# CLIAI/speaker-diarization-toolkit

Hardware: AMD Instinct MI355X
Metric: segment-embeddings/sec (higher is better)
Workload: dtype bf16; 1 GPU; config #2: 1k synthetic 2-s segments/GPU -> fbank -> ECAPA-TDNN C=1024 -> L2 -> cosine argmax vs 100 profiles; segments_per_gpu=1000, embed_dim=192, weights=random-init seed 0 (20.77 M params), parallelism=segments sharded x1, profiles replicated

## Files before the change

### speaker-diarization-toolkit_amd/csrc/common.hpp

```cpp
#pragma once
#include <hip/hip_runtime.h>
#include <stdint.h>
#include <stdio.h>
#include <vector>

#include "../../include/sdk_hip.h"

typedef __bf16 bf16_t;
typedef __bf16 bf16x8 __attribute__((ext_vector_type(8)));
typedef __bf16 bf16x4 __attribute__((ext_vector_type(4)));
typedef __bf16 bf16x2 __attribute__((ext_vector_type(2)));
typedef float f32x4 __attribute__((ext_vector_type(4)));
typedef float f32x16 __attribute__((ext_vector_type(16)));
typedef uint32_t u32x4 __attribute__((ext_vector_type(4)));
typedef uint32_t u32x2 __attribute__((ext_vector_type(2)));

struct sdk_prof_rec {
  int family;
  hipEvent_t a, b;
  double flops, bytes;
};
struct sdk_ctx {
  int device;
  int num_cu;
  hipDeviceProp_t prop;
  bool prof_on = false;
  bool no_chain_fusion = false;
  bool no_chain_two_per_cu = false;
  bool no_chain_packed = false;
  bool no_asp_packed = false;
  bool no_asp_seg = false;
  bool no_h_kblocked = false;
  int precision = 0;
  int aff_fast = 1;
  void* dbg_ptr = nullptr;
  void* gemm_clk_ptr = nullptr;
  void* gemm_stamps_ptr = nullptr;
  int hp_gemm_variant = 0;
  int matvec_variant = 0;
  int aff_boundary_pen = 0;
  int chol_pivot_rtol_ppb = 1000;
  int chol_shift_ppb = 0;
  bool ahc_distances_only = false;
  bool snorm_scores_only = false;
  int aff_variant = 0;
  std::vector<const void*> lds_optin;
  std::vector<sdk_prof_rec> prof;
};

int sdk_lds_optin(sdk_ctx* ctx, const void* func, int bytes);

int asp_fused_launch(sdk_ctx* ctx, const uint16_t* ah, int64_t ldah, const uint16_t* w2, const uint16_t* w2p, const float* b2,
                     const uint16_t* h, int64_t ldh, int B, int T, int C, int A, float* pooled, void* stream, bool kblocked = false, bool f16 = false);

int se_gate_residual_impl(sdk_ctx* ctx, const uint16_t* z, int64_t ldz, const uint16_t* x, int64_t ldx, const float* w1t, const float* b1, const float* w2t,
                          const float* b2, uint16_t* out, int64_t ldo, int B, int T, int C, int Cse, const float* mean_in, void* ws, size_t ws_bytes,
                          void* stream, bool f16);
int asp_stats_impl(sdk_ctx* ctx, const uint16_t* h, int64_t ldh, int B, int T, int C, float* out_ctx, void* stream, bool f16);
int asp_pool_impl(sdk_ctx* ctx, const float* logits, int64_t ldl, const uint16_t* h, int64_t ldh, int B, int T, int C, float* pooled, void* stream, bool f16);

int res2net_chain_launch(sdk_ctx* ctx, const uint16_t* U, int64_t ldu, uint16_t* R, int64_t ldr, const uint16_t* const* W,
                         const uint16_t* const* Wpk, const float* const* bias, const float* const* scale, const float* const* shift,
                         int nconv, int B, int T, int dil, void* stream, bool f16 = false);

int resnet_tstp_impl(sdk_ctx* ctx, const uint16_t* x, int B, int F, int T, int C, float* out, void* stream, bool f16);
int resnet_masked_tstp_impl(sdk_ctx* ctx, const uint16_t* x, int B, int F, int T, int C, int S, const float* w, const int32_t* valid, float* out,
                            void* stream, bool f16);
int resnet_zero_invalid_impl(sdk_ctx* ctx, float* emb, int n, int dim, const int32_t* valid, void* stream);

size_t ahc_workspace_bytes(const int32_t* offsets, int G);
int ahc_launch(sdk_ctx* ctx, const float* E, int ldE, int dim, const int32_t* offsets, int G, double* Z, int32_t* status, void* ws, void* stream);

struct ProfScope {
  sdk_ctx* c; hipStream_t s; size_t slot; bool on;
  ProfScope(sdk_ctx* ctx, void* stream, int family, double flops, double bytes) : c(ctx), s((hipStream_t)stream), slot(0), on(ctx && ctx->prof_on) {
    if (!on) return;
    sdk_prof_rec r{family, nullptr, nullptr, flops, bytes};
    (void)hipEventCreate(&r.a); (void)hipEventCreate(&r.b);
    (void)hipEventRecord(r.a, s);
    slot = c->prof.size();
    c->prof.push_back(r);
  }
  ~ProfScope() { if (on) (void)hipEventRecord(c->prof[slot].b, s); }
};

void sdk_set_error(const char* fmt, ...) __attribute__((format(printf, 1, 2)));

#define SDK_HIP_OK(expr)                                                              \
  do {                                                                                \
    hipError_t _e = (expr);                                                           \
    if (_e != hipSuccess) {                                                           \
      sdk_set_error("%s failed: %s (%s:%d)", #expr, hipGetErrorString(_e), __FILE__, __LINE__); \
      return 1;                                                                       \
    }                                                                                 \
  } while (0)

#define SDK_REQUIRE(cond, ...)            \
  do {                                    \
    if (!(cond)) {                        \
      sdk_set_error(__VA_ARGS__);         \
      return 2;                           \
    }                                     \
  } while (0)

#define SDK_LAUNCH_CHECK()                                                         \
  do {                                                                             \
    hipError_t _e = hipGetLastError();                                             \
    if (_e != hipSuccess) {                                                        \
      sdk_set_error("kernel launch failed: %s (%s:%d)", hipGetErrorString(_e), __FILE__, __LINE__); \
      return 1;                                                                    \
    }                                                                              \
  } while (0)

static inline int ceil_div(int a, int b) { return (a + b - 1) / b; }

__device__ __forceinline__ float bf16_to_f32(bf16_t v) { return (float)v; }
__device__ __forceinline__ bf16_t f32_to_bf16(float v) { return (bf16_t)v; }

__device__ __forceinline__ float bf16_bits_to_f32(uint32_t lo16) { return __uint_as_float(lo16 << 16); }

__device__ __forceinline__ void unpack8(const u32x4& v, float* f) {
#pragma unroll
  for (int i = 0; i < 4; ++i) {
    f[2 * i] = __uint_as_float(v[i] << 16);
    f[2 * i + 1] = __uint_as_float(v[i] & 0xffff0000u);
  }
}
__device__ __forceinline__ uint32_t pack2(float a, float b) {
  bf16x2 t;
  t[0] = (bf16_t)a;
  t[1] = (bf16_t)b;
  return __builtin_bit_cast(uint32_t, t);
}
typedef _Float16 f16x8_t __attribute__((ext_vector_type(8)));
typedef _Float16 f16x2_t __attribute__((ext_vector_type(2)));
__device__ __forceinline__ float sat_f16(float a) {
  const float c = fminf(fmaxf(a, -65504.f), 65504.f);
  return a != a ? a : c;
}
template <bool F16>
__device__ __forceinline__ uint32_t pack2t(float a, float b) {
  if constexpr (F16) {
    f16x2_t t;
    t[0] = (_Float16)sat_f16(a);
    t[1] = (_Float16)sat_f16(b);
    return __builtin_bit_cast(uint32_t, t);
  } else {
    return pack2(a, b);
  }
}
template <bool F16>
__device__ __forceinline__ void unpack8t(const u32x4& v, float* f) {
  if constexpr (F16) {
#pragma unroll
    for (int i = 0; i < 4; ++i) {
      const uint32_t w = v[i];
      const f16x2_t t = __builtin_bit_cast(f16x2_t, w);
      f[2 * i] = (float)t[0];
      f[2 * i + 1] = (float)t[1];
    }
  } else {
    unpack8(v, f);
  }
}

__device__ __forceinline__ u32x4 pack8(const float* f) {
  u32x4 v;
#pragma unroll
  for (int i = 0; i < 4; ++i) v[i] = pack2(f[2 * i], f[2 * i + 1]);
  return v;
}
template <bool F16>
__device__ __forceinline__ u32x4 pack8t(const float* f) {
  u32x4 v;
#pragma unroll
  for (int i = 0; i < 4; ++i) v[i] = pack2t<F16>(f[2 * i], f[2 * i + 1]);
  return v;
}
template <bool F16>
__device__ __forceinline__ float load1t(const bf16_t* q) {
  if constexpr (F16) return (float)*reinterpret_cast<const _Float16*>(q);
  else return bf16_to_f32(*q);
}
template <bool F16>
__device__ __forceinline__ f32x4 mfma_16x16x32(bf16x8 a, bf16x8 b, f32x4 c) {
  if constexpr (F16) return __builtin_amdgcn_mfma_f32_16x16x32_f16(__builtin_bit_cast(f16x8_t, a), __builtin_bit_cast(f16x8_t, b), c, 0, 0, 0);
  else return __builtin_amdgcn_mfma_f32_16x16x32_bf16(a, b, c, 0, 0, 0);
}
template <bool F16>
__device__ __forceinline__ f32x16 mfma_32x32x16(bf16x8 a, bf16x8 b, f32x16 c) {
  if constexpr (F16) return __builtin_amdgcn_mfma_f32_32x32x16_f16(__builtin_bit_cast(f16x8_t, a), __builtin_bit_cast(f16x8_t, b), c, 0, 0, 0);
  else return __builtin_amdgcn_mfma_f32_32x32x16_bf16(a, b, c, 0, 0, 0);
}

__device__ __forceinline__ float wave_sum(float v) {
#pragma unroll
  for (int o = 32; o > 0; o >>= 1) v += __shfl_xor(v, o, 64);
  return v;
// ... 25 lines not shown
```

### speaker-diarization-toolkit_amd/csrc/fbank.hip

```cpp
#include <math.h>
#include <string.h>

#include <type_traits>

#include "common.hpp"
#include "hp.hpp"

namespace {

constexpr int NFFT = 400, HOP = 160, NMEL = 80, NBIN = 201;
constexpr int FT = 32;
constexpr int NW = 7;
constexpr int NSYM = 208;
constexpr int KSTEPS = NSYM / 16;
constexpr int TILE_SAMPLES = (FT - 1) * HOP + NFFT;
constexpr int AROW = NSYM + 8;
constexpr int PW_STRIDE = NW * 32 + 1;
constexpr int MELW_MAX = 512;

struct FbankTables {
  uint16_t dft[NW][2][KSTEPS][2][64][8];
  int32_t mstart[NMEL];
  int32_t mlen[NMEL];
  int32_t moff[NMEL];
  float melw[MELW_MAX];
  uint16_t dft16[NW][2][KSTEPS][2][64][8];
};

template <bool F16>
__global__ __launch_bounds__(NW * 64) __attribute__((amdgpu_waves_per_eu(4, 4))) void fbank_tile_kernel(const int16_t* __restrict__ pcm, int S, int T,
                                                            int tiles_per_seg, const FbankTables* __restrict__ tab,
                                                            float* __restrict__ L, unsigned long long* __restrict__ dbg,
                                                            const int32_t* __restrict__ starts, int64_t n_total) {
  __shared__ __attribute__((aligned(16))) char lds[4 * FT * AROW * 2 + TILE_SAMPLES * 4];
  int nstamp = 0;
  auto stamp = [&]() { if (dbg && threadIdx.x == 0 && blockIdx.x < 256) dbg[blockIdx.x * 16 + nstamp++] = __builtin_amdgcn_s_memrealtime(); };
  stamp();
  typedef typename std::conditional<F16, _Float16, bf16_t>::type el_t;
  typedef el_t elx8 __attribute__((ext_vector_type(8)));
  typedef el_t elx2 __attribute__((ext_vector_type(2)));
  el_t* img = reinterpret_cast<el_t*>(lds);
  float* xs = reinterpret_cast<float*>(lds + 4 * FT * AROW * 2);
  float* pw = reinterpret_cast<float*>(lds);
  static_assert(FT * PW_STRIDE * 4 <= 4 * FT * AROW * 2, "power tile must fit over the folded images");
  static_assert((MELW_MAX + 3 * NMEL) * 4 <= TILE_SAMPLES * 4, "mel tables must fit over the raw samples");
  const int tid = threadIdx.x, lane = tid & 63, w = tid >> 6;
  const int b = blockIdx.x / tiles_per_seg;
  const int t0 = (blockIdx.x - b * tiles_per_seg) * FT;
  const int64_t s0 = (int64_t)t0 * HOP - NFFT / 2;
  const int64_t w0 = starts ? (int64_t)starts[b] : (int64_t)b * S;
  const int16_t* seg = pcm + w0;
  const int Sv = starts ? (int)(n_total - w0 < S ? (n_total - w0 < 0 ? 0 : n_total - w0) : S) : S;

  {
    constexpr int NLD = (TILE_SAMPLES + NW * 64 - 1) / (NW * 64);
    int16_t raw[NLD];
#pragma unroll
    for (int i = 0; i < NLD; ++i) {
      const int64_t g = s0 + tid + i * (NW * 64);
      raw[i] = seg[g < 0 ? 0 : (g < Sv ? g : (Sv > 0 ? Sv - 1 : 0))];
    }
#pragma unroll
    for (int i = 0; i < NLD; ++i) {
      const int q = tid + i * (NW * 64);
      const int64_t g = s0 + q;
      if (q < TILE_SAMPLES) xs[q] = (g >= 0 && g < Sv) ? (float)raw[i] * (1.0f / 32768.0f) : 0.f;
    }
  }
  __syncthreads();
  stamp();
  for (int e = tid; e < FT * (NSYM / 2); e += NW * 64) {
    const int i = e / (NSYM / 2), n = (e - i * (NSYM / 2)) * 2;
    float ec[2] = {0.f, 0.f}, es[2] = {0.f, 0.f};
#pragma unroll
    for (int q = 0; q < 2; ++q) {
      const int nn = n + q;
      if (nn <= NFFT / 2) {
        const float xa = xs[i * HOP + nn], xb = xs[i * HOP + (nn == 0 ? 0 : NFFT - nn)];
        ec[q] = xa + xb;
        es[q] = xa - xb;
      }
    }
    const el_t ch0 = (el_t)ec[0], ch1 = (el_t)ec[1], sh0 = (el_t)es[0], sh1 = (el_t)es[1];
    auto pk = [](float a, float b) { elx2 t; t[0] = (el_t)a; t[1] = (el_t)b; return __builtin_bit_cast(uint32_t, t); };
    uint32_t* dst = reinterpret_cast<uint32_t*>(img + i * AROW + n);
    dst[(0 * FT * AROW) / 2] = pk((float)ch0, (float)ch1);
    dst[(1 * FT * AROW) / 2] = pk(ec[0] - (float)ch0, ec[1] - (float)ch1);
    dst[(2 * FT * AROW) / 2] = pk((float)sh0, (float)sh1);
    dst[(3 * FT * AROW) / 2] = pk(es[0] - (float)sh0, es[1] - (float)sh1);
  }
  __syncthreads();
  stamp();

  f32x16 are, aim;
#pragma unroll
  for (int r = 0; r < 16; ++r) { are[r] = 0.f; aim[r] = 0.f; }
  const int fi = lane & 31, kk = lane >> 5;
  const el_t* arow = img + fi * AROW + kk * 8;
  const __amdgpu_buffer_rsrc_t trs = __builtin_amdgcn_make_buffer_rsrc(const_cast<uint16_t*>(F16 ? &tab->dft16[0][0][0][0][0][0] : &tab->dft[0][0][0][0][0][0]), 0, (int)sizeof(tab->dft), 0x00020000);
  const int wu = __builtin_amdgcn_readfirstlane(w);
  elx8 bt[3][4];
  elx8 ac[2][4];
  auto load_b = [&](int ks, elx8* dst) {
#pragma unroll
    for (int v = 0; v < 2; ++v) {
      dst[v] = __builtin_bit_cast(elx8, __builtin_amdgcn_raw_buffer_load_b128(trs, lane * 16, ((((wu * 2 + 0) * KSTEPS + ks) * 2 + v) * 64) * 16, 0));
      dst[2 + v] = __builtin_bit_cast(elx8, __builtin_amdgcn_raw_buffer_load_b128(trs, lane * 16, ((((wu * 2 + 1) * KSTEPS + ks) * 2 + v) * 64) * 16, 0));
    }
  };
  auto load_a = [&](int ks, elx8* dst) {
#pragma unroll
    for (int q = 0; q < 4; ++q) dst[q] = *reinterpret_cast<const elx8*>(arow + (q * FT) * AROW + ks * 16);
  };
  auto mma = [](const elx8& a, const elx8& b, const f32x16& c) {
    if constexpr (F16) return __builtin_amdgcn_mfma_f32_32x32x16_f16(a, b, c, 0, 0, 0);
    else return __builtin_amdgcn_mfma_f32_32x32x16_bf16(a, b, c, 0, 0, 0);
  };
  load_b(0, bt[0]);
  load_b(1, bt[1]);
  load_a(0, ac[0]);
#pragma unroll
  for (int ks = 0; ks < KSTEPS; ++ks) {
    __builtin_amdgcn_sched_barrier(0);
    if (ks + 2 < KSTEPS) load_b(ks + 2, bt[(ks + 2) % 3]);
    if (ks + 1 < KSTEPS) load_a(ks + 1, ac[(ks + 1) & 1]);
    __builtin_amdgcn_sched_barrier(0);
    const elx8* bc = bt[ks % 3];
    const elx8* aa = ac[ks & 1];
    are = mma(aa[1], bc[0], are);
    aim = mma(aa[3], bc[2], aim);
    are = mma(aa[0], bc[1], are);
    aim = mma(aa[2], bc[3], aim);
    are = mma(aa[0], bc[0], are);
    aim = mma(aa[2], bc[2], aim);
  }
  __syncthreads();
#pragma unroll
  for (int r = 0; r < 16; ++r) {
    const int frame = (r & 3) + 8 * (r >> 2) + 4 * kk;
    pw[frame * PW_STRIDE + w * 32 + fi] = are[r] * are[r] + aim[r] * aim[r];
  }
  float* melw = xs;
  int* mtab = reinterpret_cast<int*>(xs + MELW_MAX);
  {
    constexpr int NLD = (MELW_MAX + NW * 64 - 1) / (NW * 64);
    float wv[NLD];
    int tv[3] = {0, 0, 0};
#pragma unroll
    for (int i = 0; i < NLD; ++i) wv[i] = tab->melw[min(tid + i * (NW * 64), MELW_MAX - 1)];
    if (tid < NMEL) { tv[0] = tab->mstart[tid]; tv[1] = tab->mlen[tid]; tv[2] = tab->moff[tid]; }
#pragma unroll
    for (int i = 0; i < NLD; ++i)
      if (tid + i * (NW * 64) < MELW_MAX) melw[tid + i * (NW * 64)] = wv[i];
    if (tid < NMEL) { mtab[tid] = tv[0]; mtab[NMEL + tid] = tv[1]; mtab[2 * NMEL + tid] = tv[2]; }
  }
  __syncthreads();
  stamp();
  for (int o = tid; o < FT * NMEL; o += NW * 64) {
    const int frame = o / NMEL, m = o - frame * NMEL;
    const int t = t0 + frame;
    if (t < T) {
      const int st = mtab[m], ln = mtab[NMEL + m], of = mtab[2 * NMEL + m];
      float acc = 0.f;
      for (int i = 0; i < ln; ++i) acc += pw[frame * PW_STRIDE + st + i] * melw[of + i];
      if constexpr (F16) L[((int64_t)b * T + t) * NMEL + m] = 10.0f * log10f(fmaxf(acc, 1e-10f));
      else L[((int64_t)b * T + t) * NMEL + m] = 3.0102999566398120f * __log2f(fmaxf(acc, 1e-10f));
    }
  }
  stamp();
}

template <bool HP, bool F16 = false>
__global__ __launch_bounds__(256) void fbank_norm_kernel(const float* __restrict__ L, int T, bf16_t* __restrict__ feats,
                                                        int ldf) {
  __shared__ float red[256];
  __shared__ float mean[NMEL];
  const int tid = threadIdx.x;
  const float* Ls = L + (int64_t)blockIdx.x * T * NMEL;
  float mx = -INFINITY;
  for (int i = tid; i < T * NMEL; i += 256) mx = fmaxf(mx, Ls[i]);
  red[tid] = mx;
  __syncthreads();
  for (int o = 128; o > 0; o >>= 1) {
    if (tid < o) red[tid] = fmaxf(red[tid], red[tid + o]);
    __syncthreads();
  }
  const float flo = red[0] - 80.0f;
  __syncthreads();
  const int m = tid % NMEL, g = tid / NMEL;
  const float pv = fmaxf(Ls[m], flo);
  float s = 0.f;
  if (g < 3)
    for (int t = g; t < T; t += 3) s += fmaxf(Ls[t * NMEL + m], flo) - pv;
  red[tid] = s;
  __syncthreads();
  if (tid < NMEL) mean[tid] = pv + (red[tid] + red[tid + NMEL] + red[tid + 2 * NMEL]) / (float)T;
  __syncthreads();
  const int c8n = (HP ? ldf >> 1 : ldf) >> 3;
  bf16_t* out = feats + (int64_t)blockIdx.x * T * ldf;
  for (int i = tid; i < T * c8n; i += 256) {
    const int t = i / c8n, c8 = i - t * c8n;
    float f[8];
#pragma unroll
    for (int e = 0; e < 8; ++e) {
      const int c = c8 * 8 + e;
      f[e] = c < NMEL ? fmaxf(Ls[t * NMEL + c], flo) - mean[c] : 0.f;
    }
    if constexpr (HP) sdk_hp::store8(reinterpret_cast<uint16_t*>(out) + (int64_t)t * ldf + c8 * 8, ldf >> 1, f);
    else *reinterpret_cast<u32x4*>(out + (int64_t)t * ldf + c8 * 8) = pack8t<F16>(f);
  }
}

constexpr int NORM_LDS_MAX_T = 480;
template <bool HP, bool F16 = false>
__global__ __launch_bounds__(256) void fbank_norm_lds_kernel(const float* __restrict__ L, int T, bf16_t* __restrict__ feats,
                                                            int ldf) {
  extern __shared__ __attribute__((aligned(16))) float tile[];
  __shared__ float red[256];
  __shared__ float mean[NMEL];
  const int tid = threadIdx.x;
  const int n4 = T * (NMEL / 4);
  const f32x4* Ls = reinterpret_cast<const f32x4*>(L + (int64_t)blockIdx.x * T * NMEL);
  float mx = -INFINITY;
  constexpr int UN = 8;
  for (int i0 = tid; i0 < n4; i0 += 256 * UN) {
    f32x4 v[UN];
#pragma unroll
    for (int u = 0; u < UN; ++u) v[u] = Ls[min(i0 + 256 * u, n4 - 1)];
#pragma unroll
    for (int u = 0; u < UN; ++u) {
      const int i = i0 + 256 * u;
      if (i < n4) {
        reinterpret_cast<f32x4*>(tile)[i] = v[u];
        mx = fmaxf(fmaxf(mx, fmaxf(v[u][0], v[u][1])), fmaxf(v[u][2], v[u][3]));
      }
    }
  }
  red[tid] = mx;
  __syncthreads();
  for (int o = 128; o > 0; o >>= 1) {
    if (tid < o) red[tid] = fmaxf(red[tid], red[tid + o]);
    __syncthreads();
  }
  const float flo = red[0] - 80.0f;
  __syncthreads();
  const int m = tid % NMEL, g = tid / NMEL;
  const float pv = fmaxf(tile[m], flo);
  float s = 0.f;
  if (g < 3)
    for (int t = g; t < T; t += 3) s += fmaxf(tile[t * NMEL + m], flo) - pv;
  red[tid] = s;
  __syncthreads();
  if (tid < NMEL) mean[tid] = pv + (red[tid] + red[tid + NMEL] + red[tid + 2 * NMEL]) / (float)T;
  __syncthreads();
  const int c8n = (HP ? ldf >> 1 : ldf) >> 3;
  bf16_t* out = feats + (int64_t)blockIdx.x * T * ldf;
  for (int i = tid; i < T * c8n; i += 256) {
    const int t = i / c8n, c8 = i - t * c8n;
    float f[8];
#pragma unroll
    for (int e = 0; e < 8; ++e) {
      const int c = c8 * 8 + e;
      f[e] = c < NMEL ? fmaxf(tile[t * NMEL + c], flo) - mean[c] : 0.f;
    }
    if constexpr (HP) sdk_hp::store8(reinterpret_cast<uint16_t*>(out) + (int64_t)t * ldf + c8 * 8, ldf >> 1, f);
    else *reinterpret_cast<u32x4*>(out + (int64_t)t * ldf + c8 * 8) = pack8t<F16>(f);
  }
}

}

extern "C" size_t sdk_fbank_tables_bytes(void) { return sizeof(FbankTables); }

extern "C" int sdk_fbank_tables_fill(void* host_dst, size_t bytes) {
  SDK_REQUIRE(host_dst && bytes >= sizeof(FbankTables), "sdk_fbank_tables_fill: buffer too small (%zu < %zu)", bytes,
              sizeof(FbankTables));
  FbankTables* t = (FbankTables*)host_dst;
  memset(t, 0, sizeof(FbankTables));
  const double PI = 3.14159265358979323846;
  auto bf16_bits = [](float v) -> uint16_t {
    uint32_t u;
    memcpy(&u, &v, 4);
    return (uint16_t)((u + 0x7FFFu + ((u >> 16) & 1u)) >> 16);
  };
  auto f16_bits = [](double v) -> uint16_t {
    const double a = fabs(v);
    uint16_t out;
    if (a == 0.0) out = 0;
    else {
      int e;
      (void)frexp(a, &e);
      int ex = e - 1;
      if (ex < -14) ex = -14;
      const double q = ldexp(1.0, ex - 10);
      double n = nearbyint(a / q);
      if (n >= 2048.0) { n /= 2.0; ex += 1; }
      const int mant = (int)n;
      out = mant < 1024 ? (uint16_t)mant : (uint16_t)(((ex + 15) << 10) | (mant - 1024));
    }
    return (uint16_t)(out | (v < 0 ? 0x8000u : 0u));
  };
  auto f16_val = [](uint16_t h) -> double {
    const int e = (h >> 10) & 31, m = h & 1023;
    const double a = e ? ldexp(1.0 + m / 1024.0, e - 15) : ldexp((double)m, -24);
    return (h & 0x8000u) ? -a : a;
  };
  auto bf16_val = [](uint16_t b) -> float {
    const uint32_t u = (uint32_t)b << 16;
    float v;
    memcpy(&v, &u, 4);
    return v;
  };
  for (int w = 0; w < NW; ++w)
    for (int ks = 0; ks < KSTEPS; ++ks)
      for (int l = 0; l < 64; ++l)
        for (int j = 0; j < 8; ++j) {
          const int n = ks * 16 + 8 * (l >> 5) + j;
          const int f = w * 32 + (l & 31);
          double vc = 0.0, vs = 0.0;
          if (f < NBIN && n <= NFFT / 2) {
            const double win = 0.54 - 0.46 * cos(2.0 * PI * n / NFFT);
            const double ang = 2.0 * PI * (double)((n * f) % NFFT) / NFFT;
            const double half = (n == 0 || n == NFFT / 2) ? 0.5 : 1.0;
            vc = half * win * cos(ang);
            vs = -win * sin(ang);
          }
          const uint16_t ch = bf16_bits((float)vc), sh = bf16_bits((float)vs);
          t->dft[w][0][ks][0][l][j] = ch;
          t->dft[w][0][ks][1][l][j] = bf16_bits((float)(vc - (double)bf16_val(ch)));
          t->dft[w][1][ks][0][l][j] = sh;
          t->dft[w][1][ks][1][l][j] = bf16_bits((float)(vs - (double)bf16_val(sh)));
          const uint16_t ch16 = f16_bits(vc), sh16 = f16_bits(vs);
          t->dft16[w][0][ks][0][l][j] = ch16;
          t->dft16[w][0][ks][1][l][j] = f16_bits(vc - f16_val(ch16));
          t->dft16[w][1][ks][0][l][j] = sh16;
          t->dft16[w][1][ks][1][l][j] = f16_bits(vs - f16_val(sh16));
        }
  auto hz2mel = [](double f) { return 2595.0 * log10(1.0 + f / 700.0); };
  auto mel2hz = [](double m) { return 700.0 * (pow(10.0, m / 2595.0) - 1.0); };
  double pts[NMEL + 2];
  const double mlo = hz2mel(0.0), mhi = hz2mel(8000.0);
  for (int i = 0; i < NMEL + 2; ++i) pts[i] = mel2hz(mlo + (mhi - mlo) * i / (NMEL + 1));
  int off = 0;
  for (int m = 0; m < NMEL; ++m) {
    const double lo = pts[m], ce = pts[m + 1], hi = pts[m + 2];
    int first = -1, last = -1;
    float wv[NBIN];
    for (int f = 0; f < NBIN; ++f) {
      const double fr = 8000.0 * f / (NBIN - 1);
      const double up = (fr - lo) / (ce - lo), dn = (hi - fr) / (hi - ce);
      const double v = fmax(0.0, fmin(up, dn));
      wv[f] = (float)v;
      if (v > 0.0) {
        if (first < 0) first = f;
        last = f;
      }
    }
    t->mstart[m] = first < 0 ? 0 : first;
    t->mlen[m] = first < 0 ? 0 : last - first + 1;
    t->moff[m] = off;
    SDK_REQUIRE(off + t->mlen[m] <= MELW_MAX, "sdk_fbank_tables_fill: mel table overflow");
    for (int i = 0; i < t->mlen[m]; ++i) t->melw[off + i] = wv[first + i];
    off += t->mlen[m];
  }
  return 0;
}

extern "C" size_t sdk_fbank_workspace_bytes(int B, int S) {
  if (B <= 0 || S <= 0) return 0;
  return (size_t)B * (size_t)(1 + S / HOP) * NMEL * sizeof(float);
}

static int fbank_launch(sdk_ctx* ctx, const int16_t* pcm, const int32_t* starts, int64_t n_total, int B, int S, const void* tabs, uint16_t* feats,
                        int ldf, void* ws, size_t ws_bytes, int precision, void* stream, const char* who) {
  SDK_REQUIRE(ctx && pcm && tabs && feats && ws, "%s: null argument", who);
  SDK_REQUIRE(B > 0 && S > 0, "%s: empty batch (B=%d S=%d)", who, B, S);
  SDK_REQUIRE(precision >= 0 && precision <= 2, "%s: precision=%d must be 0 (bf16), 1 (fp16 hi | lo planes) or 2 (one fp16 plane)", who, precision);
  const bool hp = precision == 1;
  if (hp) SDK_REQUIRE((ldf >> 1) >= NMEL && ldf % 16 == 0, "%s: precise mode writes planes: ldf=%d must be >= 160 and a multiple of 16", who, ldf);
  SDK_REQUIRE(ldf >= NMEL && ldf % 8 == 0, "%s: ldf=%d must be >= 80 and a multiple of 8", who, ldf);
  SDK_REQUIRE(ws_bytes >= sdk_fbank_workspace_bytes(B, S), "%s: workspace too small", who);
  SDK_REQUIRE(((uintptr_t)feats % 16) == 0 && ((uintptr_t)tabs % 16) == 0, "%s: feats/tabs must be 16-byte aligned", who);
  const int T = 1 + S / HOP;
  const int tps = ceil_div(T, FT);
  SDK_REQUIRE((int64_t)B * tps < (1ll << 31), "%s: batch too large for one launch", who);
  {
  ProfScope ps(ctx, stream, SDK_K_FBANK_TILE, 3 * 2.0 * B * T * (double)NSYM * 2 * (NW * 32) + 2.0 * B * T * NBIN * NMEL, 2.0 * B * S + 4.0 * B * T * NMEL);
  hipLaunchKernelGGL(hp ? fbank_tile_kernel<true> : fbank_tile_kernel<false>, dim3(B * tps), dim3(NW * 64), 0, (hipStream_t)stream, pcm, S, T, tps,
                     (const FbankTables*)tabs, (float*)ws, (unsigned long long*)ctx->dbg_ptr, starts, n_total);
  }
  SDK_LAUNCH_CHECK();
  ProfScope ps2(ctx, stream, SDK_K_FBANK_NORM, 3.0 * B * T * NMEL, 4.0 * B * T * NMEL + 2.0 * B * T * ldf);
  const bool f16 = precision == 2;
  void (*norm_lds)(const float*, int, bf16_t*, int) = hp ? fbank_norm_lds_kernel<true> : f16 ? fbank_norm_lds_kernel<false, true> : fbank_norm_lds_kernel<false>;
  void (*norm)(const float*, int, bf16_t*, int) = hp ? fbank_norm_kernel<true> : f16 ? fbank_norm_kernel<false, true> : fbank_norm_kernel<false>;
  if (T <= NORM_LDS_MAX_T) {
    const int lds = T * NMEL * 4;
    if (sdk_lds_optin(ctx, (const void*)norm_lds, NORM_LDS_MAX_T * NMEL * 4)) return 1;
    hipLaunchKernelGGL(norm_lds, dim3(B), dim3(256), lds, (hipStream_t)stream, (const float*)ws, T, (bf16_t*)feats, ldf);
  } else {
    hipLaunchKernelGGL(norm, dim3(B), dim3(256), 0, (hipStream_t)stream, (const float*)ws, T, (bf16_t*)feats, ldf);
  }
  SDK_LAUNCH_CHECK();
  return 0;
}

extern "C" int sdk_fbank(sdk_ctx* ctx, const int16_t* pcm, int B, int S, const void* tabs, uint16_t* feats, int ldf,
                         void* ws, size_t ws_bytes, void* stream) {
  SDK_REQUIRE(ctx, "sdk_fbank: null context");
  return fbank_launch(ctx, pcm, nullptr, 0, B, S, tabs, feats, ldf, ws, ws_bytes, ctx->precision, stream, "sdk_fbank");
}

extern "C" int sdk_fbank_fmt(sdk_ctx* ctx, const int16_t* pcm, int B, int S, const void* tabs, uint16_t* feats, int ldf,
                             void* ws, size_t ws_bytes, int precision, void* stream) {
  return fbank_launch(ctx, pcm, nullptr, 0, B, S, tabs, feats, ldf, ws, ws_bytes, precision, stream, "sdk_fbank_fmt");
}

extern "C" int sdk_fbank_windows(sdk_ctx* ctx, const int16_t* samples, int64_t n_samples, const int32_t* starts, int B, int S, const void* tabs,
                                 uint16_t* feats, int ldf, void* ws, size_t ws_bytes, void* stream) {
  SDK_REQUIRE(starts, "sdk_fbank_windows: null start table");
  SDK_REQUIRE(n_samples > 0 && n_samples < (1ll << 31), "sdk_fbank_windows: n_samples=%lld must be in [1, 2^31)", (long long)n_samples);
  SDK_REQUIRE(ctx, "sdk_fbank_windows: null context");
  return fbank_launch(ctx, samples, starts, n_samples, B, S, tabs, feats, ldf, ws, ws_bytes, ctx->precision, stream, "sdk_fbank_windows");
}

extern "C" int sdk_fbank_windows_fmt(sdk_ctx* ctx, const int16_t* samples, int64_t n_samples, const int32_t* starts, int B, int S, const void* tabs,
                                     uint16_t* feats, int ldf, void* ws, size_t ws_bytes, int precision, void* stream) {
  SDK_REQUIRE(starts, "sdk_fbank_windows_fmt: null start table");
  SDK_REQUIRE(n_samples > 0 && n_samples < (1ll << 31), "sdk_fbank_windows_fmt: n_samples=%lld must be in [1, 2^31)", (long long)n_samples);
  return fbank_launch(ctx, samples, starts, n_samples, B, S, tabs, feats, ldf, ws, ws_bytes, precision, stream, "sdk_fbank_windows_fmt");
}
```

### speaker-diarization-toolkit_amd/csrc/sdk_api.hip

```cpp
#include <stdarg.h>
#include <string.h>

#include "common.hpp"
#include "ecapa_layout.h"
#include "hp.hpp"

static thread_local char g_err[512] = "";

void sdk_set_error(const char* fmt, ...) {
  va_list ap;
  va_start(ap, fmt);
  vsnprintf(g_err, sizeof(g_err), fmt, ap);
  va_end(ap);
}

extern "C" const char* sdk_last_error(void) { return g_err; }
extern "C" int sdk_abi_version(void) { return SDK_ABI_VERSION; }

extern "C" int sdk_init(int device, sdk_ctx** out) {
  SDK_REQUIRE(out, "sdk_init: out is null");
  *out = nullptr;
  int n = 0;
  hipError_t e = hipGetDeviceCount(&n);
  if (e != hipSuccess || n <= 0) {
    sdk_set_error("sdk_init: no HIP device available (%s); this library has no CPU fallback",
                  e != hipSuccess ? hipGetErrorString(e) : "device count is 0");
    return 1;
  }
  SDK_REQUIRE(device >= 0 && device < n, "sdk_init: device %d out of range (0..%d)", device, n - 1);
  sdk_ctx* c = new sdk_ctx();
  c->device = device;
  if (hipGetDeviceProperties(&c->prop, device) != hipSuccess) {
    delete c;
    sdk_set_error("sdk_init: hipGetDeviceProperties failed");
    return 1;
  }
  if (strncmp(c->prop.gcnArchName, "gfx950", 6) != 0) {
    sdk_set_error("sdk_init: device %d is %s; libsdk_hip.so carries gfx950 (MI355X) code objects only", device,
                  c->prop.gcnArchName);
    delete c;
    return 1;
  }
  c->num_cu = c->prop.multiProcessorCount;
  SDK_HIP_OK(hipSetDevice(device));
  *out = c;
  return 0;
}

int sdk_lds_optin(sdk_ctx* ctx, const void* func, int bytes) {
  for (const void* f : ctx->lds_optin)
    if (f == func) return 0;
  SDK_HIP_OK(hipSetDevice(ctx->device));
  SDK_HIP_OK(hipFuncSetAttribute(func, hipFuncAttributeMaxDynamicSharedMemorySize, bytes));
  ctx->lds_optin.push_back(func);
  return 0;
}

extern "C" int sdk_device_malloc(sdk_ctx* ctx, size_t bytes, void** out) {
  SDK_REQUIRE(ctx && out, "sdk_device_malloc: null argument");
  *out = nullptr;
  SDK_HIP_OK(hipSetDevice(ctx->device));
  SDK_HIP_OK(hipMalloc(out, bytes ? bytes : 1));
  return 0;
}
extern "C" int sdk_device_free(sdk_ctx* ctx, void* p) {
  SDK_REQUIRE(ctx, "sdk_device_free: null context");
  if (p) SDK_HIP_OK(hipFree(p));
  return 0;
}
extern "C" int sdk_memcpy(sdk_ctx* ctx, void* dst, const void* src, size_t bytes, int kind, void* stream) {
  SDK_REQUIRE(ctx && (bytes == 0 || (dst && src)), "sdk_memcpy: null argument");
  SDK_REQUIRE(kind >= 1 && kind <= 3, "sdk_memcpy: kind=%d (1 = host to device, 2 = device to host, 3 = device to device)", kind);
  if (!bytes) return 0;
  const hipMemcpyKind k = kind == 1 ? hipMemcpyHostToDevice : kind == 2 ? hipMemcpyDeviceToHost : hipMemcpyDeviceToDevice;
  SDK_HIP_OK(hipMemcpyAsync(dst, src, bytes, k, (hipStream_t)stream));
  SDK_HIP_OK(hipStreamSynchronize((hipStream_t)stream));
  return 0;
}
extern "C" int sdk_stream_synchronize(sdk_ctx* ctx, void* stream) {
  SDK_REQUIRE(ctx, "sdk_stream_synchronize: null context");
  SDK_HIP_OK(hipStreamSynchronize((hipStream_t)stream));
  return 0;
}

extern "C" int sdk_shutdown(sdk_ctx* ctx) {
  delete ctx;
  return 0;
}

extern "C" int sdk_get_device_info(sdk_ctx* ctx, sdk_device_info* out) {
  SDK_REQUIRE(ctx && out, "sdk_get_device_info: null argument");
  memset(out, 0, sizeof(*out));
  out->device = ctx->device;
  out->compute_units = ctx->prop.multiProcessorCount;
  out->clock_khz = ctx->prop.clockRate;
  out->wavefront_size = ctx->prop.warpSize;
  out->hbm_bytes = ctx->prop.totalGlobalMem;
  strncpy(out->name, ctx->prop.name, sizeof(out->name) - 1);
  strncpy(out->arch, ctx->prop.gcnArchName, sizeof(out->arch) - 1);
  return 0;
}

extern "C" int sdk_set_option(sdk_ctx* ctx, const char* name, int value) {
  SDK_REQUIRE(ctx && name, "sdk_set_option: null argument");
  if (strcmp(name, "res2net_chain_fusion") == 0) { ctx->no_chain_fusion = value == 0; return 0; }
  if (strcmp(name, "res2net_packed_weights") == 0) { ctx->no_chain_packed = value == 0; return 0; }
  if (strcmp(name, "res2net_two_per_cu") == 0) { ctx->no_chain_two_per_cu = value == 0; return 0; }
  if (strcmp(name, "asp_packed_weights") == 0) { ctx->no_asp_packed = value == 0; return 0; }
  if (strcmp(name, "asp_per_segment") == 0) { ctx->no_asp_seg = value == 0; return 0; }
  if (strcmp(name, "h_kblocked") == 0) { ctx->no_h_kblocked = value == 0; return 0; }
  if (strcmp(name, "precision") == 0) {
    SDK_REQUIRE(value >= 0 && value <= 2, "sdk_set_option: precision must be 0 (bf16 operands), 1 (fp16 hi+lo planes) or 2 (one fp16 plane), got %d", value);
    ctx->precision = value;
    return 0;
  }
  if (strcmp(name, "gemm_variant") == 0) return sdk_set_gemm_variant(value);
  if (strcmp(name, "affinity_fast_path") == 0) { ctx->aff_fast = value; return 0; }
  if (strcmp(name, "affinity_variant") == 0) { ctx->aff_variant = value; return 0; }
  if (strcmp(name, "affinity_boundary_penalty") == 0) { ctx->aff_boundary_pen = value < 0 ? 0 : value; return 0; }
  if (strcmp(name, "matvec_variant") == 0) { ctx->matvec_variant = value; return 0; }
  if (strcmp(name, "hp_gemm_variant") == 0) { ctx->hp_gemm_variant = value; return 0; }
  if (strcmp(name, "affinity_whole_groups") == 0) return 0;
  if (strcmp(name, "chol_pivot_rtol_ppb") == 0) { ctx->chol_pivot_rtol_ppb = value < 0 ? 0 : value; return 0; }
  if (strcmp(name, "chol_shift_ppb") == 0) { ctx->chol_shift_ppb = value < 0 ? 0 : value; return 0; }
  if (strcmp(name, "ahc_distances_only") == 0) { ctx->ahc_distances_only = value != 0; return 0; }
  if (strcmp(name, "snorm_scores_only") == 0) { ctx->snorm_scores_only = value != 0; return 0; }
  sdk_set_error("sdk_set_option: unknown option '%s'", name);
  return 2;
}

extern "C" int sdk_debug_set_ptr(sdk_ctx* ctx, const char* name, void* p) {
  SDK_REQUIRE(ctx && name, "sdk_debug_set_ptr: null argument");
  if (strcmp(name, "stamps") == 0) { ctx->dbg_ptr = p; return 0; }
  if (strcmp(name, "gemm_clock") == 0) { ctx->gemm_clk_ptr = p; return 0; }
  if (strcmp(name, "gemm_stamps") == 0) { ctx->gemm_stamps_ptr = p; return 0; }
  sdk_set_error("sdk_debug_set_ptr: unknown name '%s'", name);
  return 2;
}

extern "C" int sdk_profile_begin(sdk_ctx* ctx) {
  SDK_REQUIRE(ctx, "sdk_profile_begin: null ctx");
  for (auto& r : ctx->prof) { (void)hipEventDestroy(r.a); (void)hipEventDestroy(r.b); }
  ctx->prof.clear();
  ctx->prof_on = true;
  return 0;
}

extern "C" int sdk_profile_end(sdk_ctx* ctx, sdk_profile_report* out) {
  SDK_REQUIRE(ctx && out, "sdk_profile_end: null argument");
  ctx->prof_on = false;
  memset(out, 0, sizeof(*out));
  SDK_HIP_OK(hipDeviceSynchronize());
  for (auto& r : ctx->prof) {
    float ms = 0.f;
    SDK_HIP_OK(hipEventElapsedTime(&ms, r.a, r.b));
    if (r.family >= 0 && r.family < SDK_K_COUNT) {
      out->launches[r.family] += 1;
      out->ms[r.family] += ms;
      out->flops[r.family] += r.flops;
      out->bytes[r.family] += r.bytes;
    }
    (void)hipEventDestroy(r.a);
    (void)hipEventDestroy(r.b);
  }
  ctx->prof.clear();
  return 0;
}

namespace {

inline size_t a256(size_t v) { return (v + 255) & ~(size_t)255; }

struct FwdWs {
  uint16_t *X0, *U, *R, *Z, *Sa, *Sb, *CAT, *H, *AH;
  float *ctx, *ubias, *logits, *pooled, *se, *stats, *mean;
};

size_t fwd_layout(const sdk_ecapa_desc* d, int B, int T, char* base, FwdWs* w) {
  const size_t M = (size_t)B * T, C = d->channels, Cm = d->mfa_channels, S = d->sub_channels, A = d->attn_channels;
  size_t off = 0;
  auto take = [&](size_t bytes) { char* p = base ? base + off : nullptr; off += a256(bytes); return p; };
  char* x0 = take(M * C * 2);
  char* u = take(M * C * 2);
  char* r = take(M * C * 2);
  char* z = take(M * C * 2);
  char* sa = take(M * S * 2);
  char* sb = take(M * S * 2);
  char* cat = take(M * Cm * 2);
  char* h = take(M * Cm * 2);
  char* ah = take(M * A * 2);
  char* cx = take((size_t)B * 2 * Cm * 4);
  char* ub = take((size_t)B * A * 4);
  const bool fused_asp = A == 128 && T <= sdk_asp_fused_max_frames();
  char* lg = take(fused_asp ? 256 : M * Cm * 4);
  char* po = take((size_t)B * 2 * Cm * 4);
  char* se = take(sdk_se_workspace_bytes(B, (int)C, d->se_channels));
  char* stp = take(sdk_conv_gemm_stats_bytes((int)M, (int)Cm, 2));
  char* mn = take((size_t)B * C * 4);
  if (w) { w->se = (float*)se; w->stats = (float*)stp; w->mean = (float*)mn; }
  if (w) {
    w->X0 = (uint16_t*)x0; w->U = (uint16_t*)u; w->R = (uint16_t*)r; w->Z = (uint16_t*)z;
    w->Sa = (uint16_t*)sa; w->Sb = (uint16_t*)sb; w->CAT = (uint16_t*)cat; w->H = (uint16_t*)h; w->AH = (uint16_t*)ah;
    w->ctx = (float*)cx; w->ubias = (float*)ub; w->logits = (float*)lg; w->pooled = (float*)po;
  }
  return off;
}

struct FwdWsHp {
  uint16_t *X0, *U, *R, *Z, *Sa, *Sb, *CAT, *H, *AH;
  float *ctx, *ubias, *logits, *pooled, *mean, *hid, *gate;
};

size_t fwd_layout_hp(const sdk_ecapa_desc* d, int B, int T, char* base, FwdWsHp* w) {
  const size_t M = (size_t)B * T, C = d->channels, Cm = d->mfa_channels, S = d->sub_channels, A = d->attn_channels;
  size_t off = 0;
  auto take = [&](size_t bytes) { char* p = base ? base + off : nullptr; off += a256(bytes); return p; };
  char* x0 = take(M * C * 4);
  char* u = take(M * C * 4);
  char* r = take(M * C * 4);
  char* z = take(M * C * 4);
  char* sa = take(M * S * 4);
  char* sb = take(M * S * 4);
  char* cat = take(M * Cm * 4);
  char* h = take(M * Cm * 4);
  char* ah = take(M * A * 4);
  char* cx = take((size_t)B * 2 * Cm * 4);
  char* ub = take((size_t)B * A * 4);
  char* lg = take(M * Cm * 4);
  char* po = take((size_t)B * 2 * Cm * 4);
  char* mn = take((size_t)B * C * 4);
  char* hd = take((size_t)B * d->se_channels * 4);
  char* gt = take((size_t)B * C * 4);
  if (w) {
    w->X0 = (uint16_t*)x0; w->U = (uint16_t*)u; w->R = (uint16_t*)r; w->Z = (uint16_t*)z; w->Sa = (uint16_t*)sa; w->Sb = (uint16_t*)sb;
    w->CAT = (uint16_t*)cat; w->H = (uint16_t*)h; w->AH = (uint16_t*)ah; w->ctx = (float*)cx; w->ubias = (float*)ub; w->logits = (float*)lg;
    w->pooled = (float*)po; w->mean = (float*)mn; w->hid = (float*)hd; w->gate = (float*)gt;
  }
  return off;
}

int check_desc(const sdk_ecapa_desc* d) {
  SDK_REQUIRE(d, "ecapa desc is null");
  SDK_REQUIRE(d->n_blocks >= 1 && d->n_blocks <= 4, "ecapa desc: n_blocks=%d", d->n_blocks);
  SDK_REQUIRE(d->channels % 128 == 0 && d->mfa_channels == d->n_blocks * d->channels, "ecapa desc: channels=%d mfa=%d", d->channels, d->mfa_channels);
  SDK_REQUIRE(d->scale >= 2 && d->sub_channels * d->scale == d->channels && d->sub_channels % 128 == 0, "ecapa desc: res2net scale=%d sub=%d", d->scale, d->sub_channels);
  SDK_REQUIRE(d->attn_channels % 128 == 0 && d->n_mels_padded % (d->precision == 1 ? 32 : 64) == 0, "ecapa desc: attn=%d mels=%d", d->attn_channels, d->n_mels_padded);
  SDK_REQUIRE((d->kernel0 & 1) == 1, "ecapa desc: kernel0=%d must be odd", d->kernel0);
  SDK_REQUIRE(d->precision >= 0 && d->precision <= 2, "ecapa desc: precision=%d", d->precision);
  return 0;
}

int ecapa_forward_hp(sdk_ctx* ctx, const void* wblob, const sdk_ecapa_desc* d, const uint16_t* feats, int ldf, int B, int T, void* ws,
                     float* emb, void* stream) {
  FwdWsHp w;
  fwd_layout_hp(d, B, T, (char*)ws, &w);
  const char* wb = (const char*)wblob;
  auto P16 = [&](int slot) -> const uint16_t* { return d->off[slot] < 0 ? nullptr : (const uint16_t*)(wb + d->off[slot]); };
  auto P32 = [&](int slot) -> const float* { return d->off[slot] < 0 ? nullptr : (const float*)(wb + d->off[slot]); };
  const int M = B * T, C = d->channels, Cm = d->mfa_channels, S = d->sub_channels, A = d->attn_channels;
  const int flo = ldf >> 1;
  SDK_REQUIRE(ldf % 16 == 0 && flo >= d->n_mels_padded, "sdk_ecapa_forward: precise mode takes feature planes, ldf=%d must be >= 2 x %d", ldf, d->n_mels_padded);

  auto tdnn = [&](const uint16_t* Ain, int64_t lda, int64_t a_lo, int Cin, int taps, int dil, int slot, int N, uint16_t* Cout, int64_t ldc, int64_t c_lo,
                  const uint16_t* X2, int64_t ldx2, int64_t x2_lo, uint16_t* Sout, int64_t lds, int64_t s_lo) -> int {
    sdk_conv_gemm_hp_args g;
    memset(&g, 0, sizeof(g));
    g.A = Ain; g.lda = lda; g.a_lo = a_lo; g.W = P16(slot + EL_W); g.C = Cout; g.ldc = ldc; g.c_lo = c_lo;
    g.bias = P32(slot + EL_B); g.scale = P32(slot + EL_SCALE); g.shift = P32(slot + EL_SHIFT);
    g.X2 = X2; g.ldx2 = ldx2; g.x2_lo = x2_lo; g.S = Sout; g.lds = lds; g.s_lo = s_lo;
    g.M = M; g.N = N; g.Cin = Cin; g.taps = taps; g.dil = dil; g.T = T; g.flags = SDK_GEMM_RELU;
    SDK_REQUIRE(g.W && g.bias && g.scale && g.shift, "sdk_ecapa_forward: weight slot %d missing", slot);
    return sdk_conv_gemm_hp(ctx, &g, stream);
  };
  hipStream_t st = (hipStream_t)stream;
// ... 494 lines not shown
```

Baseline: 121,800 segment-embeddings/sec.

## Add persistent fbank tile kernel that prefetches next tile's PCM during compute

Adds a persistent variant of the fbank tile kernel, enabled by default, with a grid of two workgroups per CU that loop over tiles. Mel weights and DFT table prefetch are loaded once per workgroup, and the next tile's PCM samples are requested into registers while the current tile's DFT MFMA and mel stages run. This targets per-workgroup launch and setup cost and global load latency in the fbank stage. It adds register pressure and fixes occupancy at four waves per EU. Fbank is probably a small share of the full ECAPA pipeline, so the end-to-end effect may be small.

```diff
diff --git a/speaker-diarization-toolkit_amd/csrc/common.hpp b/speaker-diarization-toolkit_amd/csrc/common.hpp
--- a/speaker-diarization-toolkit_amd/csrc/common.hpp
+++ b/speaker-diarization-toolkit_amd/csrc/common.hpp
@@ -44,6 +44,7 @@
   bool ahc_distances_only = false;
   bool snorm_scores_only = false;
   int aff_variant = 0;
+  int fbank_variant = 1;
   std::vector<const void*> lds_optin;
   std::vector<sdk_prof_rec> prof;
 };
diff --git a/speaker-diarization-toolkit_amd/csrc/fbank.hip b/speaker-diarization-toolkit_amd/csrc/fbank.hip
--- a/speaker-diarization-toolkit_amd/csrc/fbank.hip
+++ b/speaker-diarization-toolkit_amd/csrc/fbank.hip
@@ -1,6 +1,7 @@
 #include <math.h>
 #include <string.h>
 
+#include <algorithm>
 #include <type_traits>
 
 #include "common.hpp"
@@ -168,6 +169,179 @@
     }
   }
   stamp();
+}
+
+constexpr int MEL_LDS = (MELW_MAX + 3 * NMEL) * 4;
+template <bool F16>
+__global__ __launch_bounds__(NW * 64) __attribute__((amdgpu_waves_per_eu(4, 4))) void fbank_tile_persistent_kernel(
+    const int16_t* __restrict__ pcm, int S, int T, int tiles_per_seg, int n_tiles, const FbankTables* __restrict__ tab, float* __restrict__ L,
+    unsigned long long* __restrict__ dbg, const int32_t* __restrict__ starts, int64_t n_total) {
+  __shared__ __attribute__((aligned(16))) char lds[4 * FT * AROW * 2 + TILE_SAMPLES * 4 + MEL_LDS];
+  static_assert(2 * sizeof(lds) <= 160 * 1024, "two workgroups per CU");
+  int nstamp = 0;
+  auto stamp = [&]() { if (dbg && threadIdx.x == 0 && blockIdx.x < 256 && nstamp < 2 + 3 * 4) dbg[blockIdx.x * 16 + nstamp++] = __builtin_amdgcn_s_memrealtime(); };
+  stamp();
+  typedef typename std::conditional<F16, _Float16, bf16_t>::type el_t;
+  typedef el_t elx8 __attribute__((ext_vector_type(8)));
+  typedef el_t elx2 __attribute__((ext_vector_type(2)));
+  el_t* img = reinterpret_cast<el_t*>(lds);
+  float* xs = reinterpret_cast<float*>(lds + 4 * FT * AROW * 2);
+  float* pw = reinterpret_cast<float*>(lds);
+  float* melw = reinterpret_cast<float*>(lds + 4 * FT * AROW * 2 + TILE_SAMPLES * 4);
+  int* mtab = reinterpret_cast<int*>(melw + MELW_MAX);
+  const int tid = threadIdx.x, lane = tid & 63, w = tid >> 6;
+  constexpr int NLD = (TILE_SAMPLES + NW * 64 - 1) / (NW * 64);
+
+  struct TileAt { int b, t0, Sv; int64_t s0; const int16_t* seg; };
+  auto tile_at = [&](int tile) {
+    TileAt a;
+    a.b = tile / tiles_per_seg;
+    a.t0 = (tile - a.b * tiles_per_seg) * FT;
+    a.s0 = (int64_t)a.t0 * HOP - NFFT / 2;
+    const int64_t w0 = starts ? (int64_t)starts[a.b] : (int64_t)a.b * S;
+    a.Sv = starts ? (int)(n_total - w0 < S ? (n_total - w0 < 0 ? 0 : n_total - w0) : S) : S;
+    a.seg = a.Sv > 0 ? pcm + w0 : pcm;
+    return a;
+  };
+  int16_t raw[NLD];
+  auto request = [&](const TileAt& a, int tid) {
+#pragma unroll
+    for (int i = 0; i < NLD; ++i) {
+      const int64_t g = a.s0 + tid + i * (NW * 64);
+      raw[i] = a.seg[g < 0 ? 0 : (g < a.Sv ? g : (a.Sv > 0 ? a.Sv - 1 : 0))];
+    }
+  };
+  auto convert = [&](const TileAt& a, int tid) {
+#pragma unroll
+    for (int i = 0; i < NLD; ++i) {
+      const int q = tid + i * (NW * 64);
+      const int64_t g = a.s0 + q;
+      if (q < TILE_SAMPLES) xs[q] = (g >= 0 && g < a.Sv) ? (float)raw[i] * (1.0f / 32768.0f) : 0.f;
+    }
+  };
+
+  const __amdgpu_buffer_rsrc_t trs = __builtin_amdgcn_make_buffer_rsrc(const_cast<uint16_t*>(F16 ? &tab->dft16[0][0][0][0][0][0] : &tab->dft[0][0][0][0][0][0]), 0, (int)sizeof(tab->dft), 0x00020000);
+  const int wu = __builtin_amdgcn_readfirstlane(w);
+  const int fi = lane & 31, kk = lane >> 5;
+  const el_t* arow = img + fi * AROW + kk * 8;
+  elx8 bt[3][4];
+  elx8 ac[2][4];
+  auto load_b = [&](int ks, elx8* dst, int wu) {
+#pragma unroll
+    for (int v = 0; v < 2; ++v) {
+      dst[v] = __builtin_bit_cast(elx8, __builtin_amdgcn_raw_buffer_load_b128(trs, lane * 16, ((((wu * 2 + 0) * KSTEPS + ks) * 2 + v) * 64) * 16, 0));
+      dst[2 + v] = __builtin_bit_cast(elx8, __builtin_amdgcn_raw_buffer_load_b128(trs, lane * 16, ((((wu * 2 + 1) * KSTEPS + ks) * 2 + v) * 64) * 16, 0));
+    }
+  };
+  auto load_a = [&](int ks, elx8* dst) {
+#pragma unroll
+    for (int q = 0; q < 4; ++q) dst[q] = *reinterpret_cast<const elx8*>(arow + (q * FT) * AROW + ks * 16);
+  };
+  auto mma = [](const elx8& a, const elx8& b, const f32x16& c) {
+    if constexpr (F16) return __builtin_amdgcn_mfma_f32_32x32x16_f16(a, b, c, 0, 0, 0);
+    else return __builtin_amdgcn_mfma_f32_32x32x16_bf16(a, b, c, 0, 0, 0);
+  };
+
+  int tile = blockIdx.x;
+  TileAt cur = tile_at(tile);
+  request(cur, tid);
+  load_b(0, bt[1], wu);
+  load_b(1, bt[2], wu);
+  {
+    constexpr int NMW = (MELW_MAX + NW * 64 - 1) / (NW * 64);
+    float wv[NMW];
+    int tv[3] = {0, 0, 0};
+#pragma unroll
+    for (int i = 0; i < NMW; ++i) wv[i] = tab->melw[min(tid + i * (NW * 64), MELW_MAX - 1)];
+    if (tid < NMEL) { tv[0] = tab->mstart[tid]; tv[1] = tab->mlen[tid]; tv[2] = tab->moff[tid]; }
+#pragma unroll
+    for (int i = 0; i < NMW; ++i)
+      if (tid + i * (NW * 64) < MELW_MAX) melw[tid + i * (NW * 64)] = wv[i];
+    if (tid < NMEL) { mtab[tid] = tv[0]; mtab[NMEL + tid] = tv[1]; mtab[2 * NMEL + tid] = tv[2]; }
+  }
+  convert(cur, tid);
+  lds_barrier();
+  stamp();
+
+  for (; tile < n_tiles; tile += gridDim.x) {
+    const bool has_next = tile + gridDim.x < n_tiles;
+    const TileAt nxt = tile_at(has_next ? tile + gridDim.x : n_tiles - 1);
+    int tf = tid;
+    asm volatile("" : "+v"(tf));
+    request(nxt, tf);
+    for (int e = tf; e < FT * (NSYM / 2); e += NW * 64) {
+      const int i = e / (NSYM / 2), n = (e - __mul24(i, NSYM / 2)) * 2;
+      float ec[2] = {0.f, 0.f}, es[2] = {0.f, 0.f};
+#pragma unroll
+      for (int q = 0; q < 2; ++q) {
+        const int nn = n + q;
+        if (nn <= NFFT / 2) {
+          const float xa = xs[__mul24(i, HOP) + nn], xb = xs[__mul24(i, HOP) + (nn == 0 ? 0 : NFFT - nn)];
+          ec[q] = xa + xb;
+          es[q] = xa - xb;
+        }
+      }
+      const el_t ch0 = (el_t)ec[0], ch1 = (el_t)ec[1], sh0 = (el_t)es[0], sh1 = (el_t)es[1];
+      auto pk = [](float a, float b) { elx2 t; t[0] = (el_t)a; t[1] = (el_t)b; return __builtin_bit_cast(uint32_t, t); };
+      uint32_t* dst = reinterpret_cast<uint32_t*>(img + __mul24(i, AROW) + n);
+      dst[(0 * FT * AROW) / 2] = pk((float)ch0, (float)ch1);
+      dst[(1 * FT * AROW) / 2] = pk(ec[0] - (float)ch0, ec[1] - (float)ch1);
+      dst[(2 * FT * AROW) / 2] = pk((float)sh0, (float)sh1);
+      dst[(3 * FT * AROW) / 2] = pk(es[0] - (float)sh0, es[1] - (float)sh1);
+    }
+    lds_barrier();
+    stamp();
+    if (has_next) convert(nxt, tf);
+
+    f32x16 are, aim;
+#pragma unroll
+    for (int r = 0; r < 16; ++r) { are[r] = 0.f; aim[r] = 0.f; }
+#pragma unroll
+    for (int q = 0; q < 4; ++q) { bt[0][q] = bt[1][q]; bt[1][q] = bt[2][q]; }
+    int wt = wu;
+    asm volatile("" : "+s"(wt));
+    load_a(0, ac[0]);
+#pragma unroll
+    for (int ks = 0; ks < KSTEPS; ++ks) {
+      __builtin_amdgcn_sched_barrier(0);
+      load_b((ks + 2) % KSTEPS, bt[(ks + 2) % 3], wt);
+      if (ks + 1 < KSTEPS) load_a(ks + 1, ac[(ks + 1) & 1]);
+      __builtin_amdgcn_sched_barrier(0);
+      const elx8* bc = bt[ks % 3];
+      const elx8* aa = ac[ks & 1];
+      are = mma(aa[1], bc[0], are);
+      aim = mma(aa[3], bc[2], aim);
+      are = mma(aa[0], bc[1], are);
+      aim = mma(aa[2], bc[3], aim);
+      are = mma(aa[0], bc[0], are);
+      aim = mma(aa[2], bc[2], aim);
+    }
+    lds_barrier();
+    stamp();
+#pragma unroll
+    for (int r = 0; r < 16; ++r) {
+      const int frame = (r & 3) + 8 * (r >> 2) + 4 * kk;
+      pw[frame * PW_STRIDE + w * 32 + fi] = are[r] * are[r] + aim[r] * aim[r];
+    }
+    lds_barrier();
+    stamp();
+    int tm = tid;
+    asm volatile("" : "+v"(tm));
+    for (int o = tm; o < FT * NMEL; o += NW * 64) {
+      const int frame = o / NMEL, m = o - frame * NMEL;
+      const int t = cur.t0 + frame;
+      if (t < T) {
+        const int st = mtab[m], ln = mtab[NMEL + m], of = mtab[2 * NMEL + m];
+        float acc = 0.f;
+        for (int i = 0; i < ln; ++i) acc += pw[frame * PW_STRIDE + st + i] * melw[of + i];
+        if constexpr (F16) L[((int64_t)cur.b * T + t) * NMEL + m] = 10.0f * log10f(fmaxf(acc, 1e-10f));
+        else L[((int64_t)cur.b * T + t) * NMEL + m] = 3.0102999566398120f * __log2f(fmaxf(acc, 1e-10f));
+      }
+    }
+    lds_barrier();
+    stamp();
+    cur = nxt;
+  }
 }
 
 template <bool HP, bool F16 = false>
@@ -386,8 +560,14 @@
   SDK_REQUIRE((int64_t)B * tps < (1ll << 31), "%s: batch too large for one launch", who);
   {
   ProfScope ps(ctx, stream, SDK_K_FBANK_TILE, 3 * 2.0 * B * T * (double)NSYM * 2 * (NW * 32) + 2.0 * B * T * NBIN * NMEL, 2.0 * B * S + 4.0 * B * T * NMEL);
-  hipLaunchKernelGGL(hp ? fbank_tile_kernel<true> : fbank_tile_kernel<false>, dim3(B * tps), dim3(NW * 64), 0, (hipStream_t)stream, pcm, S, T, tps,
-                     (const FbankTables*)tabs, (float*)ws, (unsigned long long*)ctx->dbg_ptr, starts, n_total);
+  if (ctx->fbank_variant == 0) {
+    hipLaunchKernelGGL(hp ? fbank_tile_kernel<true> : fbank_tile_kernel<false>, dim3(B * tps), dim3(NW * 64), 0, (hipStream_t)stream, pcm, S, T, tps,
+                       (const FbankTables*)tabs, (float*)ws, (unsigned long long*)ctx->dbg_ptr, starts, n_total);
+  } else {
+    const int n_tiles = B * tps, grid = std::min(n_tiles, 2 * (ctx->num_cu > 0 ? ctx->num_cu : 256));
+    hipLaunchKernelGGL(hp ? fbank_tile_persistent_kernel<true> : fbank_tile_persistent_kernel<false>, dim3(grid), dim3(NW * 64), 0, (hipStream_t)stream, pcm,
+                       S, T, tps, n_tiles, (const FbankTables*)tabs, (float*)ws, (unsigned long long*)ctx->dbg_ptr, starts, n_total);
+  }
   }
   SDK_LAUNCH_CHECK();
   ProfScope ps2(ctx, stream, SDK_K_FBANK_NORM, 3.0 * B * T * NMEL, 4.0 * B * T * NMEL + 2.0 * B * T * ldf);
diff --git a/speaker-diarization-toolkit_amd/csrc/sdk_api.hip b/speaker-diarization-toolkit_amd/csrc/sdk_api.hip
--- a/speaker-diarization-toolkit_amd/csrc/sdk_api.hip
+++ b/speaker-diarization-toolkit_amd/csrc/sdk_api.hip
@@ -120,6 +120,11 @@
   if (strcmp(name, "affinity_boundary_penalty") == 0) { ctx->aff_boundary_pen = value < 0 ? 0 : value; return 0; }
   if (strcmp(name, "matvec_variant") == 0) { ctx->matvec_variant = value; return 0; }
   if (strcmp(name, "hp_gemm_variant") == 0) { ctx->hp_gemm_variant = value; return 0; }
+  if (strcmp(name, "fbank_variant") == 0) {
+    SDK_REQUIRE(value == 0 || value == 1, "sdk_set_option: fbank_variant must be 0 (one workgroup per tile) or 1 (persistent workgroups), got %d", value);
+    ctx->fbank_variant = value;
+    return 0;
+  }
   if (strcmp(name, "affinity_whole_groups") == 0) return 0;
   if (strcmp(name, "chol_pivot_rtol_ppb") == 0) { ctx->chol_pivot_rtol_ppb = value < 0 ? 0 : value; return 0; }
   if (strcmp(name, "chol_shift_ppb") == 0) { ctx->chol_shift_ppb = value < 0 ? 0 : value; return 0; }
```

After: 120,100 segment-embeddings/sec. 1.4% lower.
